# vsergeev/luaradio

Measured on AMD Instinct MI355X. Metric: MSamples/s per block (128-tap complex FIR headline) + WBFM chain end-to-end, higher is better.
Workload: dtype f32

## Files before the change

luaradio_amd/csrc/kernels_channelizer.h:

```cpp
#pragma once
#include "common.h"
#include "kernels_fir.h"

#ifndef LRHIP_CHAN_EXP
#define LRHIP_CHAN_EXP 0
#endif

namespace lrhip {

#ifndef LRHIP_CHAN_INTERLEAVE
#define LRHIP_CHAN_INTERLEAVE 1
#endif
#ifndef LRHIP_CHAN_RT
#define LRHIP_CHAN_RT 1
#endif
#ifndef LRHIP_CHAN_KSLAB
#define LRHIP_CHAN_KSLAB 32
#endif
constexpr int CHAN_RT = LRHIP_CHAN_RT;
constexpr int CHAN_MT = 64 * CHAN_RT;
constexpr int CHAN_KSLAB = LRHIP_CHAN_KSLAB;

template <int NCT>
__global__ __launch_bounds__(256, CHAN_RT == 1 ? 2 : 1) void channelizer_kernel(const float *__restrict__ hist, const float *__restrict__ x,
                                                             const float *__restrict__ W, float *__restrict__ y,
                                                             int M, long n, long nframes, long first)
{
    constexpr int K2 = 16 * NCT;
    constexpr int K = K2 / 2;
    constexpr int DROW = K2 + 2;
    constexpr int WROW = K2 + 16;
    extern __shared__ __attribute__((aligned(16))) float lds[];
    const int tid = threadIdx.x, lane = tid & 63, wave = tid >> 6;
    const int col = lane & 15, kq = lane >> 4;
    const long f0 = (long)blockIdx.x * CHAN_MT;
    const int nsamp = (CHAN_MT - 1) * K + M;
    const int nflt = 2 * nsamp;
    float *ldsD = lds;
    const int dsize = ((nflt + 2 * (nflt / K2) + 2 + 3) / 4) * 4;
    float *ldsW = lds + dsize;

    const long p0 = first + f0 * K;
    const long xlo = p0 - (M - 1);
    if (xlo >= 0 && xlo + nsamp <= n && ((reinterpret_cast<uintptr_t>(x + 2 * xlo) & 15) == 0)) {
        const float4 *src = reinterpret_cast<const float4 *>(x + 2 * xlo);
        for (int i4 = tid; i4 < nflt / 4; i4 += 256) {
            float4 v = src[i4];
            int a = 4 * i4, p = a + 2 * (a / K2);
            *reinterpret_cast<float2 *>(ldsD + p) = make_float2(v.x, v.y);
            *reinterpret_cast<float2 *>(ldsD + p + 2) = make_float2(v.z, v.w);
        }
        for (int a = (nflt / 4) * 4 + tid; a < nflt; a += 256) ldsD[a + 2 * (a / K2)] = x[2 * xlo + a];
    } else {
        for (int r = tid; r < nsamp; r += 256) {
            int a = 2 * r, p = a + 2 * (a / K2);
            ldsD[p] = stream_at<2>(hist, x, p0 + r, 0, M, n);
            ldsD[p + 1] = stream_at<2>(hist, x, p0 + r, 1, M, n);
        }
    }

    constexpr int SLAB_F4 = CHAN_KSLAB * K2 / 4;
    constexpr int UW = (SLAB_F4 + 255) / 256;
    const float4 *W4 = reinterpret_cast<const float4 *>(W);
    static_assert(UW <= 8, "W slab prefetch: at most 8 float4 per thread");
    float4 w0, w1, w2, w3, w4, w5, w6, w7;
#define LR_CHAN_FOR8(OP) OP(0) OP(1) OP(2) OP(3) OP(4) OP(5) OP(6) OP(7)
#define LR_CHAN_LOAD(U)                                                                          \
    if (U < UW) {                                                                                \
        int i4 = tid + U * 256;                                                                  \
        w##U = W4[wbase + (i4 < SLAB_F4 ? i4 : SLAB_F4 - 1)];                                    \
    }
#define LR_CHAN_PUT(U)                                                                           \
    if (U < UW) {                                                                                \
        int i4 = tid + U * 256;                                                                  \
        if (i4 < SLAB_F4) *reinterpret_cast<float4 *>(wdst + ((4 * i4) / K2) * WROW + (4 * i4) % K2) = w##U; \
    }
    {
        const size_t wbase = 0;
        float *wdst = ldsW;
        LR_CHAN_FOR8(LR_CHAN_LOAD)
        LR_CHAN_FOR8(LR_CHAN_PUT)
    }
    __syncthreads();

    f32x4 acc[CHAN_RT][NCT];
#pragma unroll
    for (int r = 0; r < CHAN_RT; r++)
#pragma unroll
        for (int c = 0; c < NCT; c++) acc[r][c] = (f32x4){0.f, 0.f, 0.f, 0.f};
    const float *abase = ldsD + DROW * (wave * 16 * CHAN_RT + col) + kq;
    const int nslabs = 2 * M / CHAN_KSLAB;
    for (int s = 0; s < nslabs; s++) {
        const float *wcur = ldsW + (s & 1) * (CHAN_KSLAB * WROW);
#if LRHIP_CHAN_EXP == 1
        const bool more = false;
#else
        const bool more = s + 1 < nslabs;
#endif
        if (more) {
            const size_t wbase = (size_t)(s + 1) * SLAB_F4;
            LR_CHAN_FOR8(LR_CHAN_LOAD)
        }
        const float *ap = abase + CHAN_KSLAB * s + 2 * ((CHAN_KSLAB * s) / K2);
        const float *bp = wcur + kq * WROW + col;
        constexpr int NST = CHAN_KSLAB / 4;
        float av[2][CHAN_RT], bv[2][NCT];
        auto fetch = [&](int buf, int st) {
#pragma unroll
            for (int r = 0; r < CHAN_RT; r++) av[buf][r] = ap[16 * r * DROW + 4 * st];
#pragma unroll
            for (int c = 0; c < NCT; c++) bv[buf][c] = bp[4 * st * WROW + 16 * c];
        };
        fetch(0, 0);
#pragma unroll
        for (int st = 0; st < NST; st++) {
#if LRHIP_CHAN_INTERLEAVE
            if (st + 1 < NST) fetch((st + 1) & 1, st + 1);
#pragma unroll
            for (int c = 0; c < NCT; c++)
#pragma unroll
                for (int r = 0; r < CHAN_RT; r++)
                    acc[r][c] = __builtin_amdgcn_mfma_f32_16x16x4f32(av[st & 1][r], bv[st & 1][c], acc[r][c], 0, 0, 0);
#pragma unroll
            for (int i = 0; i < NCT * CHAN_RT; i++) {
                __builtin_amdgcn_sched_group_barrier(0x008, 1, 0);
                __builtin_amdgcn_sched_group_barrier(0x100, 1, 0);
            }
            __builtin_amdgcn_sched_barrier(0);
#else
            if (st + 1 < NST) fetch((st + 1) & 1, st + 1);
            __builtin_amdgcn_sched_barrier(0);
#pragma unroll
            for (int c = 0; c < NCT; c++)
#pragma unroll
                for (int r = 0; r < CHAN_RT; r++)
                    acc[r][c] = __builtin_amdgcn_mfma_f32_16x16x4f32(av[st & 1][r], bv[st & 1][c], acc[r][c], 0, 0, 0);
            __builtin_amdgcn_sched_barrier(0);
#endif
        }
        if (more) {
            float *wdst = ldsW + ((s + 1) & 1) * (CHAN_KSLAB * WROW);
            LR_CHAN_FOR8(LR_CHAN_PUT)
        }
#if LRHIP_CHAN_EXP != 1
        __syncthreads();
#endif
    }

#pragma unroll
    for (int rt = 0; rt < CHAN_RT; rt++)
#pragma unroll
        for (int c = 0; c < NCT; c++)
#pragma unroll
            for (int r = 0; r < 4; r++) {
                long f = f0 + (wave * CHAN_RT + rt) * 16 + 4 * kq + r;
                if (f < nframes) y[f * K2 + 16 * c + col] = acc[rt][c][r];
            }
}

#undef LR_CHAN_FOR8
#undef LR_CHAN_LOAD
#undef LR_CHAN_PUT

}
```

luaradio_amd/csrc/lrhip.hip:

```cpp
#include "../../include/lrhip.h"

#include <cmath>
#include <map>
#include <memory>
#include <string>

#include "common.h"
#include "kernels_elem.h"
#include "kernels_fft.h"
#include "kernels_fir.h"
#include "kernels_firfft.h"
#include "kernels_firdecfft.h"
#include "kernels_firdecim.h"
#include "kernels_channelizer.h"
#include "kernels_pfb.h"
#include "kernels_iir.h"
#include "kernels_agc.h"
#include "kernels_firwin.h"
#include "kernels_firwin2.h"
#include "kernels_firfft4k.h"
#include "kernels_firpols.h"
#include "kernels_firfft64.h"
#include "kernels_interp.h"
#include "kernels_rx.h"
#include "kernels_digital.h"
#include "kernels_bitscan.h"
#include "kernels_preamble.h"
#include "kernels_rdsframer.h"
#include "kernels_ertframer.h"
#include "kernels_ax25framer.h"
#include "kernels_pocsagframer.h"
#include "kernels_phasecorr.h"
#include "kernels_modulator.h"
#include "kernels_pll.h"

using namespace lrhip;

static int g_launches = 0;
#define LR_LAUNCH_CHECK()                                                                              \
    do {                                                                                               \
        g_launches++;                                                                                  \
        hipError_t e__ = hipGetLastError();                                                            \
        if (e__ != hipSuccess) return set_error("kernel launch failed: %s (%s:%d)", hipGetErrorString(e__), __FILE__, __LINE__); \
    } while (0)

#include "stage.h"
#include "stage_counted.h"
#include "stage_fir.h"
#include "stage_elem.h"
#include "stage_iir.h"
#include "stage_firwin.h"
#include "stage_spectrum.h"
#include "stage_elem2.h"
#include "stage_resample.h"
#include "stage_pfb.h"
#include "stage_elem3.h"
#include "stage_rx.h"
#include "chain.h"
#include "stage_phasecorr.h"
#include "stage_digital.h"
#include "stage_pll.h"
#include "stage_preamble.h"
#include "stage_framers.h"
#include "stage_modulator.h"
#include "chain_plan.h"

extern "C" {

const char *lrhip_version(void) { return "lrhip 0.1 (gfx950)"; }
const char *lrhip_strerror(void) { return err_buf(); }

int lrhip_init(int device)
{
    err_buf()[0] = 0;
    return ensure_init(device);
}

int lrhip_device(void)
{
    const Context &c = ctx();
    return (c.ready && c.pid == (long)getpid()) ? c.device : -1;
}

int lrhip_device_count(void)
{
    if (ctx().ready && ctx().pid != (long)getpid()) return ensure_init();
    int count = 0;
    LR_HIP(hipGetDeviceCount(&count));
    return count;
}

int lrhip_set_stream(void *hip_stream)
{
    if (ensure_init()) return -1;
    hipStream_t next = hip_stream == (void *)1 ? (hipStream_t) nullptr : hip_stream ? (hipStream_t)hip_stream : ctx().own_stream, prev = ctx().stream;
    if (next != prev) {
        hipEvent_t ev = nullptr;
// ... 284 lines not shown
    if (q->reset()) return nullptr;
    return q.release();
}

lrhip_stage_t *lrhip_unary_create(const char *op, float re, float im, int constant_complex, int input_complex)
{
    if (!op) { set_error("unary: missing operation name"); return nullptr; }
    {
        std::string name;
        std::map<std::string, double> kv;
        const char *c = strchr(op, ':');
        const std::string head(op, c ? (size_t)(c - op) : strlen(op));
        if (head == "preamblesampler") return preamblesampler_create(op);
        if (head == "pam" || head == "qam") return modulator_create(op);
        if (head == "pll") return pll_create(op);
        if (head == "rdsframer") return plain_create<RfStage>(op, 8);
        if (head == "scmframer") return plain_create<EfStage<EF_SCM>>(op, EfProto<EF_SCM>::REC);
        if (head == "scmplusframer") return plain_create<EfStage<EF_SCMPLUS>>(op, EfProto<EF_SCMPLUS>::REC);
        if (head == "idmframer") return plain_create<EfStage<EF_IDM>>(op, EfProto<EF_IDM>::REC);
        if (head == "ax25framer") return plain_create<AxStage>(op, AX_REC);
        if (head == "pocsagframer") return plain_create<PgStage>(op, PG_REC);
        if (head == "manchesterdecoder") {
            if (!parse_op(op, name, kv, {"invert"})) return nullptr;
            return manchesterdecoder_create(kv, op);
        }
        if (c || digital_unary_op(head)) {
            if (!digital_unary_op(head)) { set_error("unary: unknown operation \"%s\"", op); return nullptr; }
            if (!parse_op(op, name, kv, digital_keys(head))) return nullptr;
            return digital_unary_create(name, kv, op);
        }
    }
    struct { const char *name; int code, in, out; } T[] = {
        {"complexmagnitude", UN_CMAG, 8, 4}, {"complexphase", UN_CPHASE, 8, 4}, {"complextoreal", UN_CREAL, 8, 4},
        {"complextoimag", UN_CIMAG, 8, 4},   {"complexconjugate", UN_CCONJ, 8, 8}, {"realtocomplex", UN_R2C, 4, 8},
        {"absolutevalue", UN_ABS, 4, 4}};
    int code = -1, in = 0, out = 0;
    for (auto &t : T)
        if (!strcmp(t.name, op)) { code = t.code; in = t.in; out = t.out; }
    if (!strcmp(op, "addconstant")) {
        if (constant_complex && !input_complex) { set_error("addconstant: a complex constant takes ComplexFloat32 input only (addconstant.lua:42-44)"); return nullptr; }
        code = !input_complex ? UN_ADDC_REAL : (constant_complex ? UN_ADDC_CPLX : UN_ADDC_CPLX_BY_REAL);
        in = out = input_complex ? 8 : 4;
    }
    if (code < 0) { set_error("unary: unknown operation \"%s\"", op); return nullptr; }
    if (ensure_init()) return nullptr;
    UnaryStage *q = new (std::nothrow) UnaryStage();
    if (!q) { set_error("out of memory"); return nullptr; }
    q->op = code; q->cr = re; q->ci = im;
    q->in_size = in; q->out_size = out;
    return q;
}

lrhip_stage_t *lrhip_delay_create(unsigned num_samples, int elem_size)
{
    if (num_samples < 1) { set_error("Number of samples must be greater than 0"); return nullptr; }
    if (elem_size != 4 && elem_size != 8) { set_error("delay: element size must be 4 or 8"); return nullptr; }
    if (ensure_init()) return nullptr;
    std::unique_ptr<DelayStage> q(new (std::nothrow) DelayStage());
    if (!q) { set_error("out of memory"); return nullptr; }
    q->D = num_samples;
    q->in_size = q->out_size = elem_size;
    if (q->reset()) return nullptr;
    return q.release();
}

lrhip_stage_t *lrhip_hilbert_create(const float *taps, unsigned ntaps)
{
    if (!taps || (ntaps % 2) != 1) { set_error("Number of taps must be odd"); return nullptr; }
    std::unique_ptr<HilbertStage> q(new (std::nothrow) HilbertStage());
    if (!q) { set_error("out of memory"); return nullptr; }
    q->fir.reset(fir_build(taps, ntaps, 0, 0, 1, 0, false, 0.0));
    if (!q->fir) return nullptr;
    q->in_size = 4; q->out_size = 8;
    return q.release();
}

lrhip_stage_t *lrhip_channelizer_create(const float *taps, unsigned ntaps, unsigned nchannels)
{
    if (!taps || ntaps < 32 || (ntaps % 32) != 0 || ntaps > 8192) { set_error("channelizer: ntaps must be a multiple of 32 in [32, 8192]"); return nullptr; }
    if (nchannels != 32 && nchannels != 64) { set_error("channelizer: nchannels must be 32 or 64"); return nullptr; }
    if (ensure_init()) return nullptr;
    std::unique_ptr<ChannelizerStage> q(new (std::nothrow) ChannelizerStage());
    if (!q) { set_error("out of memory"); return nullptr; }
    int M = (int)ntaps, K = (int)nchannels, K2 = 2 * K;
    q->M = M; q->K = K;
    q->in_size = q->out_size = 8;
    std::vector<float> W((size_t)2 * M * K2);
    const double PI2 = 6.283185307179586476925286766559;
    for (int i = 0; i < M; i++)
        for (int c = 0; c < K; c++) {
            int j = M - 1 - i;
            double a = PI2 * (double)(((long)c * j) % K) / K, h = taps[j];
            float gr = (float)(h * std::cos(a)), gi = (float)(h * std::sin(a));
            W[(size_t)(2 * i) * K2 + 2 * c] = gr;
            W[(size_t)(2 * i + 1) * K2 + 2 * c] = -gi;
            W[(size_t)(2 * i) * K2 + 2 * c + 1] = gi;
            W[(size_t)(2 * i + 1) * K2 + 2 * c + 1] = gr;
        }
    if (upload(q->W, W.data(), W.size() * sizeof(float))) return nullptr;
    if (q->reset()) return nullptr;
    return q.release();
}

lrhip_stage_t *lrhip_pfb_channelizer_create(const float *taps, unsigned ntaps, unsigned nchannels)
{
    return lrhip_pfb_oversampled_create(taps, ntaps, nchannels, 1);
}

lrhip_stage_t *lrhip_pfb_oversampled_create(const float *taps, unsigned ntaps, unsigned nchannels, unsigned oversample)
{
    if (const char *why = PfbChannelizerStage::refusal(taps ? ntaps : 0, nchannels, oversample)) { set_error("%s", why); return nullptr; }
    if (ensure_init()) return nullptr;
    std::unique_ptr<PfbChannelizerStage> q(new (std::nothrow) PfbChannelizerStage());
    if (!q) { set_error("out of memory"); return nullptr; }
    const int M = (int)ntaps, K = (int)nchannels;
    q->M = M; q->K = K; q->P = (M + K - 1) / K;
    q->R = (int)oversample; q->D = K / q->R;
    while ((1 << q->log2k) < K) q->log2k++;
    q->in_size = q->out_size = 8;
    std::vector<float> tw((size_t)K);
    for (int m = 0; m < K / 2; m++) {
        double ang = -2.0 * 3.14159265358979323846 * m / K;
        tw[2 * m] = (float)std::cos(ang);
        tw[2 * m + 1] = (float)std::sin(ang);
    }
    if (upload(q->taps, taps, (size_t)M * sizeof(float)) || upload(q->tw, tw.data(), tw.size() * sizeof(float))) return nullptr;
    if (q->reset()) return nullptr;
    return q.release();
}

lrhip_stage_t *lrhip_binary_create(const char *op, int input_complex)
{
    if (!op) { set_error("binary: missing operation name"); return nullptr; }
    if (!strcmp(op, "sampler")) {
        if (ensure_init()) return nullptr;
        std::unique_ptr<SamplerStage> q(new (std::nothrow) SamplerStage());
        if (!q) { set_error("out of memory"); return nullptr; }
        q->in_size = q->out_size = input_complex ? 8 : 4;
        q->in2_size = 4;
        if (q->reset()) return nullptr;
        return q.release();
    }
    int code = !strcmp(op, "multiply") ? BIN_MULTIPLY : !strcmp(op, "multiplyconjugate") ? BIN_MULTIPLY_CONJ
             : !strcmp(op, "add") ? BIN_ADD : !strcmp(op, "subtract") ? BIN_SUBTRACT : !strcmp(op, "floattocomplex") ? BIN_F2C : -1;
    if (code < 0) { set_error("binary: unknown operation \"%s\"", op); return nullptr; }
    if (code == BIN_MULTIPLY_CONJ && !input_complex) { set_error("binary: multiplyconjugate takes ComplexFloat32 inputs (multiplyconjugate.lua:26)"); return nullptr; }
    if (ensure_init()) return nullptr;
    BinaryStage *q = new (std::nothrow) BinaryStage();
    if (!q) { set_error("out of memory"); return nullptr; }
    q->op = code;
    q->in_size = q->out_size = input_complex ? 8 : 4;
    if (code == BIN_F2C) { q->in_size = 4; q->out_size = 8; }
    return q;
}

void lrhip_stage_destroy(lrhip_stage_t *q)
{
    if (!q) return;
    if (ctx().ready) (void)hipStreamSynchronize(ctx().stream);
    delete q;
}

int lrhip_stage_reset(lrhip_stage_t *q) { return q ? q->reset() : set_error("null stage"); }
int lrhip_stage_input_size(const lrhip_stage_t *q) { return q ? q->in_size : set_error("null stage"); }
int lrhip_stage_output_size(const lrhip_stage_t *q) { return q ? q->out_size : set_error("null stage"); }
unsigned long lrhip_stage_max_output(const lrhip_stage_t *q, unsigned long n_in) { return q ? q->max_output(n_in) : 0; }

long lrhip_stage_execute_device(lrhip_stage_t *q, const void *in_dev, unsigned long n_in, void *out_dev, unsigned long out_capacity)
{
    if (!q) return set_error("null stage");
    if (n_in && (!in_dev || (!out_dev && q->max_output(n_in)))) return set_error("null buffer");
    return q->run(in_dev, n_in, out_dev, out_capacity);
}

long lrhip_stage_execute(lrhip_stage_t *q, const void *in_host, unsigned long n_in, void *out_host, unsigned long out_capacity)
{
    if (!q) return set_error("null stage");
    return host_execute(q->h_in, q->h_out, q->d_in, q->d_out, q->in_size, q->out_size, q->max_output(n_in), in_host, n_in,
                        out_host, out_capacity,
                        [&](const void *di, unsigned long n, void *dout, unsigned long cap) { return q->run(di, n, dout, cap); }, q->align(), q->direct_io_ok());
}
// ... 770 lines not shown
```

luaradio_amd/csrc/stage_resample.h:

```cpp
#pragma once

struct ResampleStage : lrhip_stage {
    int S = 2, M = 0, L = 1, HQ = 0;
    unsigned long D = 1;
    float c = 1.f;
    DeviceBuf d_taps, d_ttab, hist[2];
    int cur = 0;
    uint64_t Q0 = 0, m0 = 0;
    int interp_J = 0;
    int rat_blocks_per_cu = 0;
    static bool rational_supported(int L, unsigned long D) { return (L == 3 && D == 2) || (L == 2 && D == 3) || (L == 4 && D == 3) || (L == 3 && D == 4) || (L == 5 && D == 4) || (L == 4 && D == 5); }
    int interp_blocks_per_cu = 0;
    static int resample_rounds(long ntiles, long slots)
    {
        static const char *e = getenv("LRHIP_RESAMPLE_ROUNDS");
        if (e) return atoi(e) < 0 ? 0 : atoi(e);
        return ntiles <= slots ? 0 : 1;
    }
    static constexpr int SPAN_MAX = 6144;
    const char *kind() const override { return "resample"; }
    unsigned long max_output(unsigned long n) const override { return (n * (unsigned long)L) / D + 2; }
    int seek(unsigned long long n0, unsigned long long *n0_out) override
    {
        if (reset()) return -1;
// ... 26 lines not shown
                if (!interp_blocks_per_cu) {
                    int nb = 0;
                    LR_HIP(hipOccupancyMaxActiveBlocksPerMultiprocessor(&nb, kern, FIP_NT, lds_bytes));
                    interp_blocks_per_cu = nb < 1 ? 1 : nb;
                }
                const long ntiles = ((long)n + tq - 1) / tq, slots = (long)ctx().num_cus * interp_blocks_per_cu;
                const int rounds = resample_rounds(ntiles, slots);
                const long wgs = rounds > 0 ? (ntiles + rounds - 1) / rounds : (ntiles < slots ? ntiles : slots);
                hipLaunchKernelGGL(kern, dim3((unsigned)wgs), dim3(FIP_NT), lds_bytes, ctx().stream, h, (const float *)in_dev, (const float *)d_ttab.p,
                                   (float *)out_dev, (long)n, HQ, c, ho, ablation_bits("LRHIP_INTERP_DBG"), rounds);
                return 0;
            };
#define LR_INTERP(LL, JJ) gi(fir_interp_kernel<LL, JJ>, (size_t)FipGeom<LL, JJ>::LDS_FLOATS * sizeof(float), FipGeom<LL, JJ>::TQ)
            int rc = L == 2 ? LR_INTERP(2, 64) : L == 3 ? LR_INTERP(3, 43) : L == 4 ? LR_INTERP(4, 32) : LR_INTERP(5, 26);
#undef LR_INTERP
            if (rc) return rc;
            LR_LAUNCH_CHECK();
            cur ^= 1;
            Q0 += n;
            m0 = m_end;
            return n_out;
        }
        static const bool no_rational = getenv("LRHIP_NO_RATIONAL_WIN") != nullptr;
        if (!no_rational && interp_J > 0 && D > 1 && ((uintptr_t)in_dev & 7) == 0 && ((uintptr_t)out_dev & 7) == 0) {
            auto gr = [&](auto kern, size_t lds_bytes, int tq) -> int {
                if (lds_bytes > 48 * 1024) LR_HIP(hipFuncSetAttribute((const void *)kern, hipFuncAttributeMaxDynamicSharedMemorySize, (int)lds_bytes));
                if (!rat_blocks_per_cu) {
                    int nb = 0;
                    LR_HIP(hipOccupancyMaxActiveBlocksPerMultiprocessor(&nb, kern, 256, lds_bytes));
                    rat_blocks_per_cu = nb < 1 ? 1 : nb;
                }
                const long ntiles = ((long)n + (long)(Q0 % D) + tq - 1) / tq, slots = (long)ctx().num_cus * rat_blocks_per_cu;
                const int rounds = resample_rounds(ntiles, slots);
                const long wgs = rounds > 0 ? (ntiles + rounds - 1) / rounds : (ntiles < slots ? ntiles : slots);
                hipLaunchKernelGGL(kern, dim3((unsigned)wgs), dim3(256), lds_bytes, ctx().stream, h, (const float *)in_dev, (const float *)d_ttab.p,
                                   (float *)out_dev, (long)n, n_out, m0, Q0, HQ, c, ho, rounds);
                return 0;
            };
#define LR_RAT(LL, DD, JJ, RR) gr(fir_rational_kernel<LL, DD, JJ, RR>, (size_t)FrrGeom<LL, DD, JJ, RR>::LDS_FLOATS * sizeof(float), FrrGeom<LL, DD, JJ, RR>::TQ)
            int rc = (L == 3 && D == 2) ? LR_RAT(3, 2, 43, 6) : (L == 2 && D == 3) ? LR_RAT(2, 3, 64, 9) : (L == 4 && D == 3) ? LR_RAT(4, 3, 32, 6)
                   : (L == 3 && D == 4) ? LR_RAT(3, 4, 43, 8) : (L == 5 && D == 4) ? LR_RAT(5, 4, 26, 8) : LR_RAT(4, 5, 32, 10);
#undef LR_RAT
            if (rc) return rc;
            LR_LAUNCH_CHECK();
            cur ^= 1;
            Q0 += n;
            m0 = m_end;
            return n_out;
        }
        int span_cap = (int)(256 * D / (unsigned long)L) + (M - 1) / L + 4;
        size_t lds_bytes = ((size_t)((((M - 1) / L + 1) * L + 3) & ~3) + (size_t)span_cap * S) * sizeof(float);
        auto go = [&](auto kern) -> int {
            if (lds_bytes > 48 * 1024) LR_HIP(hipFuncSetAttribute((const void *)kern, hipFuncAttributeMaxDynamicSharedMemorySize, (int)lds_bytes));
            unsigned grid = n_out > 0 ? (unsigned)((n_out + 255) / 256) : 1;
            hipLaunchKernelGGL(kern, dim3(grid), dim3(256), lds_bytes, ctx().stream, h, (const float *)in_dev, (const float *)d_taps.p, (float *)out_dev, M, L,
                               (long)D, (long)n, n_out, m0, Q0, HQ, c, span_cap, ho);
            return 0;
        };
        int rc = S == 2 ? go(fir_resample_kernel<2>) : go(fir_resample_kernel<1>);
        if (rc) return rc;
        LR_LAUNCH_CHECK();
        cur ^= 1;
        Q0 += n;
        m0 = m_end;
        return n_out;
    }
};

struct ChannelizerStage : lrhip_stage {
    int seek(unsigned long long, unsigned long long *) override { return set_error("seek: not supported by the channelizer stage"); }
    long memory() const override { return -1; }
    int M = 0, K = 0;
    DeviceBuf W, hist[2];
    int cur = 0;
    unsigned long index = 0;
    const char *kind() const override { return "channelizer"; }
    unsigned long max_output(unsigned long n) const override { return (n / K + 1) * K; }
    int reset() override
    {
        cur = 0; index = 0;
        size_t hb = (size_t)(M - 1) * 2 * sizeof(float);
        return (zero_fill(hist[0], hb) || zero_fill(hist[1], hb)) ? -1 : 0;
    }
    template <int NCT>
    int launch(const float *x, long n, float *y, long nframes)
    {
        constexpr int K2 = 16 * NCT;
        int nflt = 2 * ((CHAN_MT - 1) * K + M);
        size_t dsize = (size_t)((nflt + 2 * (nflt / K2) + 2 + 3) / 4) * 4;
        size_t lds_bytes = (dsize + (size_t)2 * CHAN_KSLAB * (K2 + 16)) * sizeof(float);
        auto kern = channelizer_kernel<NCT>;
        if (lds_bytes > 48 * 1024) LR_HIP(hipFuncSetAttribute((const void *)kern, hipFuncAttributeMaxDynamicSharedMemorySize, (int)lds_bytes));
        unsigned grid = (unsigned)((nframes + CHAN_MT - 1) / CHAN_MT);
        hipLaunchKernelGGL(kern, dim3(grid), dim3(256), lds_bytes, ctx().stream, (const float *)hist[cur].p, x, (const float *)W.p, y, M, n,
                           nframes, (long)index);
        LR_LAUNCH_CHECK();
        return 0;
    }
    long run(const void *in_dev, unsigned long n_in, void *out_dev, unsigned long cap) override
    {
        long n = (long)n_in;
        if (n <= 0) return 0;
        long nframes = n_in > index ? (long)((n_in - index + K - 1) / K) : 0;
        if ((unsigned long)(nframes * K) > cap) return set_error("channelizer: output capacity %lu < %ld", cap, nframes * K);
        const float *x = (const float *)in_dev;
        if (nframes > 0) {
            int rc = K == 32 ? launch<4>(x, n, (float *)out_dev, nframes) : launch<8>(x, n, (float *)out_dev, nframes);
            if (rc) return rc;
        }
        unsigned grid = grid_for((unsigned long)(M - 1) * 2, 256);
        hipLaunchKernelGGL(fir_history_kernel<2>, dim3(grid), dim3(256), 0, ctx().stream, (const float *)hist[cur].p, x, (float *)hist[cur ^ 1].p, M, n);
        LR_LAUNCH_CHECK();
        cur ^= 1;
        index = index + (unsigned long)nframes * K - n_in;
        return nframes * K;
    }
};
```

Before: 317,200.

## Split channelizer input into Re/Im planes and exploit real-DFT symmetry for half-size GEMM

The channelizer now splits interleaved complex input into separate real and imaginary LDS planes. It multiplies each plane by a real K-column weight matrix that holds cos for channels 0..K/2 and sin for channels 1..K/2-1, instead of a 2K-wide complex-expanded matrix. The epilogue rebuilds channels c and K-c from the four partial sums, which halves the weight matrix and the MFMA work per frame. In exchange it requires ntaps to be a multiple of the slab size and removes the multi-row-tile option.

Result: no change. 317,400, median of 3 (+0.1%).

```diff
diff --git a/luaradio_amd/csrc/kernels_channelizer.h b/luaradio_amd/csrc/kernels_channelizer.h
--- a/luaradio_amd/csrc/kernels_channelizer.h
+++ b/luaradio_amd/csrc/kernels_channelizer.h
@@ -11,60 +11,67 @@
 #ifndef LRHIP_CHAN_INTERLEAVE
 #define LRHIP_CHAN_INTERLEAVE 1
 #endif
-#ifndef LRHIP_CHAN_RT
-#define LRHIP_CHAN_RT 1
-#endif
 #ifndef LRHIP_CHAN_KSLAB
 #define LRHIP_CHAN_KSLAB 32
 #endif
-constexpr int CHAN_RT = LRHIP_CHAN_RT;
-constexpr int CHAN_MT = 64 * CHAN_RT;
+constexpr int CHAN_MT = 64;
 constexpr int CHAN_KSLAB = LRHIP_CHAN_KSLAB;
 
+__host__ __device__ constexpr int chan_tile_samples(int K, int M) { return (CHAN_MT - 1) * K + M; }
+__host__ __device__ constexpr int chan_plane_floats(int K, int M)
+{
+    return (chan_tile_samples(K, M) + 2 * (chan_tile_samples(K, M) / K) + 2 + 3) / 4 * 4;
+}
+__host__ __device__ constexpr int chan_wrow(int K) { return K + 16; }
+__host__ __device__ constexpr size_t chan_lds_bytes(int K, int M)
+{
+    return ((size_t)2 * chan_plane_floats(K, M) + (size_t)2 * CHAN_KSLAB * chan_wrow(K)) * sizeof(float);
+}
+
 template <int NCT>
-__global__ __launch_bounds__(256, CHAN_RT == 1 ? 2 : 1) void channelizer_kernel(const float *__restrict__ hist, const float *__restrict__ x,
+__global__ __launch_bounds__(256, 2) void channelizer_kernel(const float *__restrict__ hist, const float *__restrict__ x,
                                                              const float *__restrict__ W, float *__restrict__ y,
                                                              int M, long n, long nframes, long first)
 {
-    constexpr int K2 = 16 * NCT;
-    constexpr int K = K2 / 2;
-    constexpr int DROW = K2 + 2;
-    constexpr int WROW = K2 + 16;
+    constexpr int K = 16 * NCT;
+    constexpr int H = NCT / 2;
+    constexpr int DROW = K + 2;
+    constexpr int WROW = chan_wrow(K);
+    static_assert(NCT % 2 == 0, "Re and Im of a channel sit in tiles t and t + NCT/2");
+    static_assert(K % CHAN_KSLAB == 0 || CHAN_KSLAB % K == 0, "a slab starts on a plane row or stays inside one");
     extern __shared__ __attribute__((aligned(16))) float lds[];
     const int tid = threadIdx.x, lane = tid & 63, wave = tid >> 6;
     const int col = lane & 15, kq = lane >> 4;
     const long f0 = (long)blockIdx.x * CHAN_MT;
-    const int nsamp = (CHAN_MT - 1) * K + M;
-    const int nflt = 2 * nsamp;
-    float *ldsD = lds;
-    const int dsize = ((nflt + 2 * (nflt / K2) + 2 + 3) / 4) * 4;
-    float *ldsW = lds + dsize;
+    const int nsamp = chan_tile_samples(K, M);
+    const int psize = chan_plane_floats(K, M);
+    float *ldsRe = lds, *ldsIm = lds + psize;
+    float *ldsW = lds + 2 * psize;
 
     const long p0 = first + f0 * K;
     const long xlo = p0 - (M - 1);
     if (xlo >= 0 && xlo + nsamp <= n && ((reinterpret_cast<uintptr_t>(x + 2 * xlo) & 15) == 0)) {
         const float4 *src = reinterpret_cast<const float4 *>(x + 2 * xlo);
-        for (int i4 = tid; i4 < nflt / 4; i4 += 256) {
+        for (int i4 = tid; i4 < nsamp / 2; i4 += 256) {
             float4 v = src[i4];
-            int a = 4 * i4, p = a + 2 * (a / K2);
-            *reinterpret_cast<float2 *>(ldsD + p) = make_float2(v.x, v.y);
-            *reinterpret_cast<float2 *>(ldsD + p + 2) = make_float2(v.z, v.w);
+            int r = 2 * i4, p = r + 2 * (r / K);
+            *reinterpret_cast<float2 *>(ldsRe + p) = make_float2(v.x, v.z);
+            *reinterpret_cast<float2 *>(ldsIm + p) = make_float2(v.y, v.w);
         }
-        for (int a = (nflt / 4) * 4 + tid; a < nflt; a += 256) ldsD[a + 2 * (a / K2)] = x[2 * xlo + a];
     } else {
         for (int r = tid; r < nsamp; r += 256) {
-            int a = 2 * r, p = a + 2 * (a / K2);
-            ldsD[p] = stream_at<2>(hist, x, p0 + r, 0, M, n);
-            ldsD[p + 1] = stream_at<2>(hist, x, p0 + r, 1, M, n);
+            int p = r + 2 * (r / K);
+            ldsRe[p] = stream_at<2>(hist, x, p0 + r, 0, M, n);
+            ldsIm[p] = stream_at<2>(hist, x, p0 + r, 1, M, n);
         }
     }
 
-    constexpr int SLAB_F4 = CHAN_KSLAB * K2 / 4;
+    constexpr int SLAB_F4 = CHAN_KSLAB * K / 4;
     constexpr int UW = (SLAB_F4 + 255) / 256;
     const float4 *W4 = reinterpret_cast<const float4 *>(W);
-    static_assert(UW <= 8, "W slab prefetch: at most 8 float4 per thread");
-    float4 w0, w1, w2, w3, w4, w5, w6, w7;
-#define LR_CHAN_FOR8(OP) OP(0) OP(1) OP(2) OP(3) OP(4) OP(5) OP(6) OP(7)
+    static_assert(UW <= 4, "G slab prefetch: at most 4 float4 per thread");
+    float4 w0, w1, w2, w3;
+#define LR_CHAN_FOR4(OP) OP(0) OP(1) OP(2) OP(3)
 #define LR_CHAN_LOAD(U)                                                                          \
     if (U < UW) {                                                                                \
         int i4 = tid + U * 256;                                                                  \
@@ -73,23 +80,23 @@
 #define LR_CHAN_PUT(U)                                                                           \
     if (U < UW) {                                                                                \
         int i4 = tid + U * 256;                                                                  \
-        if (i4 < SLAB_F4) *reinterpret_cast<float4 *>(wdst + ((4 * i4) / K2) * WROW + (4 * i4) % K2) = w##U; \
+        if (i4 < SLAB_F4) *reinterpret_cast<float4 *>(wdst + ((4 * i4) / K) * WROW + (4 * i4) % K) = w##U; \
     }
     {
         const size_t wbase = 0;
         float *wdst = ldsW;
-        LR_CHAN_FOR8(LR_CHAN_LOAD)
-        LR_CHAN_FOR8(LR_CHAN_PUT)
+        LR_CHAN_FOR4(LR_CHAN_LOAD)
+        LR_CHAN_FOR4(LR_CHAN_PUT)
     }
     __syncthreads();
 
-    f32x4 acc[CHAN_RT][NCT];
+    f32x4 acc[2][NCT];
 #pragma unroll
-    for (int r = 0; r < CHAN_RT; r++)
+    for (int p = 0; p < 2; p++)
 #pragma unroll
-        for (int c = 0; c < NCT; c++) acc[r][c] = (f32x4){0.f, 0.f, 0.f, 0.f};
-    const float *abase = ldsD + DROW * (wave * 16 * CHAN_RT + col) + kq;
-    const int nslabs = 2 * M / CHAN_KSLAB;
+        for (int c = 0; c < NCT; c++) acc[p][c] = (f32x4){0.f, 0.f, 0.f, 0.f};
+    const float *abase = ldsRe + DROW * (wave * 16 + col) + kq;
+    const int nslabs = M / CHAN_KSLAB;
     for (int s = 0; s < nslabs; s++) {
         const float *wcur = ldsW + (s & 1) * (CHAN_KSLAB * WROW);
 #if LRHIP_CHAN_EXP == 1
@@ -99,15 +106,15 @@
 #endif
         if (more) {
             const size_t wbase = (size_t)(s + 1) * SLAB_F4;
-            LR_CHAN_FOR8(LR_CHAN_LOAD)
+            LR_CHAN_FOR4(LR_CHAN_LOAD)
         }
-        const float *ap = abase + CHAN_KSLAB * s + 2 * ((CHAN_KSLAB * s) / K2);
+        const float *ap = abase + CHAN_KSLAB * s + 2 * ((CHAN_KSLAB * s) / K);
         const float *bp = wcur + kq * WROW + col;
         constexpr int NST = CHAN_KSLAB / 4;
-        float av[2][CHAN_RT], bv[2][NCT];
+        float av[2][2], bv[2][NCT];
         auto fetch = [&](int buf, int st) {
-#pragma unroll
-            for (int r = 0; r < CHAN_RT; r++) av[buf][r] = ap[16 * r * DROW + 4 * st];
+            av[buf][0] = ap[4 * st + 2 * ((4 * st) / K)];
+            av[buf][1] = ap[4 * st + 2 * ((4 * st) / K) + psize];
 #pragma unroll
             for (int c = 0; c < NCT; c++) bv[buf][c] = bp[4 * st * WROW + 16 * c];
         };
@@ -119,10 +126,10 @@
 #pragma unroll
             for (int c = 0; c < NCT; c++)
 #pragma unroll
-                for (int r = 0; r < CHAN_RT; r++)
-                    acc[r][c] = __builtin_amdgcn_mfma_f32_16x16x4f32(av[st & 1][r], bv[st & 1][c], acc[r][c], 0, 0, 0);
+                for (int p = 0; p < 2; p++)
+                    acc[p][c] = __builtin_amdgcn_mfma_f32_16x16x4f32(av[st & 1][p], bv[st & 1][c], acc[p][c], 0, 0, 0);
 #pragma unroll
-            for (int i = 0; i < NCT * CHAN_RT; i++) {
+            for (int i = 0; i < 2 * NCT; i++) {
                 __builtin_amdgcn_sched_group_barrier(0x008, 1, 0);
                 __builtin_amdgcn_sched_group_barrier(0x100, 1, 0);
             }
@@ -133,32 +140,40 @@
 #pragma unroll
             for (int c = 0; c < NCT; c++)
 #pragma unroll
-                for (int r = 0; r < CHAN_RT; r++)
-                    acc[r][c] = __builtin_amdgcn_mfma_f32_16x16x4f32(av[st & 1][r], bv[st & 1][c], acc[r][c], 0, 0, 0);
+                for (int p = 0; p < 2; p++)
+                    acc[p][c] = __builtin_amdgcn_mfma_f32_16x16x4f32(av[st & 1][p], bv[st & 1][c], acc[p][c], 0, 0, 0);
             __builtin_amdgcn_sched_barrier(0);
 #endif
         }
         if (more) {
             float *wdst = ldsW + ((s + 1) & 1) * (CHAN_KSLAB * WROW);
-            LR_CHAN_FOR8(LR_CHAN_PUT)
+            LR_CHAN_FOR4(LR_CHAN_PUT)
         }
 #if LRHIP_CHAN_EXP != 1
         __syncthreads();
 #endif
     }
 
+    float2 *y2 = reinterpret_cast<float2 *>(y);
 #pragma unroll
-    for (int rt = 0; rt < CHAN_RT; rt++)
+    for (int t = 0; t < H; t++)
 #pragma unroll
-        for (int c = 0; c < NCT; c++)
-#pragma unroll
-            for (int r = 0; r < 4; r++) {
-                long f = f0 + (wave * CHAN_RT + rt) * 16 + 4 * kq + r;
-                if (f < nframes) y[f * K2 + 16 * c + col] = acc[rt][c][r];
+        for (int r = 0; r < 4; r++) {
+            const long f = f0 + wave * 16 + 4 * kq + r;
+            if (f >= nframes) continue;
+            const int c = 16 * t + col;
+            const float Rr = acc[0][t][r], Ir = acc[1][t][r], Ri = acc[0][t + H][r], Ii = acc[1][t + H][r];
+            if (c != 0) {
+                y2[f * K + c] = make_float2(Rr - Ii, Ir + Ri);
+                y2[f * K + (K - c)] = make_float2(Rr + Ii, Ir - Ri);
+            } else {
+                y2[f * K] = make_float2(Rr + 0.f * Ir, Ir + 0.f * Rr);
+                y2[f * K + K / 2] = make_float2(Ri + 0.f * Ii, Ii + 0.f * Ri);
             }
+        }
 }
 
-#undef LR_CHAN_FOR8
+#undef LR_CHAN_FOR4
 #undef LR_CHAN_LOAD
 #undef LR_CHAN_PUT
 
diff --git a/luaradio_amd/csrc/lrhip.hip b/luaradio_amd/csrc/lrhip.hip
--- a/luaradio_amd/csrc/lrhip.hip
+++ b/luaradio_amd/csrc/lrhip.hip
@@ -463,20 +463,17 @@
     if (ensure_init()) return nullptr;
     std::unique_ptr<ChannelizerStage> q(new (std::nothrow) ChannelizerStage());
     if (!q) { set_error("out of memory"); return nullptr; }
-    int M = (int)ntaps, K = (int)nchannels, K2 = 2 * K;
+    int M = (int)ntaps, K = (int)nchannels, Kh = K / 2;
     q->M = M; q->K = K;
     q->in_size = q->out_size = 8;
-    std::vector<float> W((size_t)2 * M * K2);
+    std::vector<float> W((size_t)M * K);
     const double PI2 = 6.283185307179586476925286766559;
     for (int i = 0; i < M; i++)
-        for (int c = 0; c < K; c++) {
+        for (int c = 0; c <= Kh; c++) {
             int j = M - 1 - i;
             double a = PI2 * (double)(((long)c * j) % K) / K, h = taps[j];
-            float gr = (float)(h * std::cos(a)), gi = (float)(h * std::sin(a));
-            W[(size_t)(2 * i) * K2 + 2 * c] = gr;
-            W[(size_t)(2 * i + 1) * K2 + 2 * c] = -gi;
-            W[(size_t)(2 * i) * K2 + 2 * c + 1] = gi;
-            W[(size_t)(2 * i + 1) * K2 + 2 * c + 1] = gr;
+            W[(size_t)i * K + c] = (float)(h * std::cos(a));
+            if (c >= 1 && c < Kh) W[(size_t)i * K + Kh + c] = (float)(h * std::sin(a));
         }
     if (upload(q->W, W.data(), W.size() * sizeof(float))) return nullptr;
     if (q->reset()) return nullptr;
diff --git a/luaradio_amd/csrc/stage_resample.h b/luaradio_amd/csrc/stage_resample.h
--- a/luaradio_amd/csrc/stage_resample.h
+++ b/luaradio_amd/csrc/stage_resample.h
@@ -135,10 +135,8 @@
     template <int NCT>
     int launch(const float *x, long n, float *y, long nframes)
     {
-        constexpr int K2 = 16 * NCT;
-        int nflt = 2 * ((CHAN_MT - 1) * K + M);
-        size_t dsize = (size_t)((nflt + 2 * (nflt / K2) + 2 + 3) / 4) * 4;
-        size_t lds_bytes = (dsize + (size_t)2 * CHAN_KSLAB * (K2 + 16)) * sizeof(float);
+        if (M % CHAN_KSLAB) return set_error("channelizer: ntaps %d is not a multiple of the %d-row slab this library was built with", M, CHAN_KSLAB);
+        size_t lds_bytes = chan_lds_bytes(16 * NCT, M);
         auto kern = channelizer_kernel<NCT>;
         if (lds_bytes > 48 * 1024) LR_HIP(hipFuncSetAttribute((const void *)kern, hipFuncAttributeMaxDynamicSharedMemorySize, (int)lds_bytes));
         unsigned grid = (unsigned)((nframes + CHAN_MT - 1) / CHAN_MT);
@@ -155,7 +153,7 @@
         if ((unsigned long)(nframes * K) > cap) return set_error("channelizer: output capacity %lu < %ld", cap, nframes * K);
         const float *x = (const float *)in_dev;
         if (nframes > 0) {
-            int rc = K == 32 ? launch<4>(x, n, (float *)out_dev, nframes) : launch<8>(x, n, (float *)out_dev, nframes);
+            int rc = K == 32 ? launch<2>(x, n, (float *)out_dev, nframes) : launch<4>(x, n, (float *)out_dev, nframes);
             if (rc) return rc;
         }
         unsigned grid = grid_for((unsigned long)(M - 1) * 2, 256);
```

## Use conjugate-symmetric paired DFT table with split real/imag planes in channelizer

Applied to the files above, without the earlier changes.

Replaces the channelizer's complex GEMM, which used a 2x-expanded interleaved real/imag weight matrix, with a paired cos/sin table of K columns. Input is deinterleaved into separate real and imaginary LDS planes. Outputs for channel c and K-c are reconstructed from four real partial sums. This roughly halves the MFMA count and the weight traffic per frame. The cost is a larger LDS footprint for the two planes and a more complex epilogue that writes output in scattered pairs.

Measured after the change: 315,900 before, 315,800 after (median of 2 runs). No clear change (-0.0%).

```diff
diff --git a/luaradio_amd/csrc/channelizer_table.h b/luaradio_amd/csrc/channelizer_table.h
--- /dev/null
+++ b/luaradio_amd/csrc/channelizer_table.h
@@ -0,0 +1,25 @@
+#pragma once
+#include <cmath>
+#include <cstddef>
+#include <vector>
+
+namespace lrhip {
+
+inline std::vector<float> channelizer_paired_table(const float *taps, int M, int K)
+{
+    std::vector<float> Wp((size_t)M * K);
+    const double PI2 = 6.283185307179586476925286766559;
+    const int H = K / 2;
+    for (int i = 0; i < M; i++) {
+        const int j = M - 1 - i;
+        const double h = taps[j];
+        float *row = Wp.data() + (size_t)i * K;
+        auto angle = [&](int c) { return PI2 * (double)(((long)c * j) % K) / K; };
+        for (int c = 0; c < H; c++) row[c] = (float)(h * std::cos(angle(c)));
+        row[H] = (float)(h * std::cos(angle(H)));
+        for (int c = 1; c < H; c++) row[H + c] = (float)(h * std::sin(angle(c)));
+    }
+    return Wp;
+}
+
+}
diff --git a/luaradio_amd/csrc/kernels_channelizer.h b/luaradio_amd/csrc/kernels_channelizer.h
--- a/luaradio_amd/csrc/kernels_channelizer.h
+++ b/luaradio_amd/csrc/kernels_channelizer.h
@@ -2,69 +2,62 @@
 #include "common.h"
 #include "kernels_fir.h"
 
-#ifndef LRHIP_CHAN_EXP
-#define LRHIP_CHAN_EXP 0
-#endif
-
 namespace lrhip {
 
-#ifndef LRHIP_CHAN_INTERLEAVE
-#define LRHIP_CHAN_INTERLEAVE 1
-#endif
-#ifndef LRHIP_CHAN_RT
-#define LRHIP_CHAN_RT 1
-#endif
-#ifndef LRHIP_CHAN_KSLAB
-#define LRHIP_CHAN_KSLAB 32
-#endif
-constexpr int CHAN_RT = LRHIP_CHAN_RT;
-constexpr int CHAN_MT = 64 * CHAN_RT;
-constexpr int CHAN_KSLAB = LRHIP_CHAN_KSLAB;
+constexpr int CHAN_MT = 64;
+constexpr int CHAN_KSLAB = 32;
 
-template <int NCT>
-__global__ __launch_bounds__(256, CHAN_RT == 1 ? 2 : 1) void channelizer_kernel(const float *__restrict__ hist, const float *__restrict__ x,
-                                                             const float *__restrict__ W, float *__restrict__ y,
+__host__ __device__ constexpr int chan_plane_floats(int nsamp, int K) { return ((nsamp + 2 * (nsamp / K) + 2 + 3) / 4) * 4; }
+__host__ __device__ constexpr size_t chan_lds_floats(int M, int K)
+{
+    return (size_t)2 * chan_plane_floats((CHAN_MT - 1) * K + M, K) + (size_t)2 * CHAN_KSLAB * (K + 16);
+}
+
+template <int NT>
+__global__ __launch_bounds__(256, 2) void channelizer_kernel(const float *__restrict__ hist, const float *__restrict__ x,
+                                                             const float *__restrict__ Wp, float *__restrict__ y,
                                                              int M, long n, long nframes, long first)
 {
-    constexpr int K2 = 16 * NCT;
-    constexpr int K = K2 / 2;
-    constexpr int DROW = K2 + 2;
-    constexpr int WROW = K2 + 16;
+    constexpr int K = 16 * NT;
+    constexpr int HT = NT / 2;
+    constexpr int DROW = K + 2;
+    constexpr int WROW = K + 16;
+    static_assert(NT == 2 || NT == 4, "K is 32 or 64");
+    static_assert(CHAN_KSLAB % 4 == 0 && K % CHAN_KSLAB == 0, "a slab lies inside one plane row");
     extern __shared__ __attribute__((aligned(16))) float lds[];
     const int tid = threadIdx.x, lane = tid & 63, wave = tid >> 6;
     const int col = lane & 15, kq = lane >> 4;
     const long f0 = (long)blockIdx.x * CHAN_MT;
     const int nsamp = (CHAN_MT - 1) * K + M;
-    const int nflt = 2 * nsamp;
-    float *ldsD = lds;
-    const int dsize = ((nflt + 2 * (nflt / K2) + 2 + 3) / 4) * 4;
-    float *ldsW = lds + dsize;
+    const int psize = chan_plane_floats(nsamp, K);
+    float *ldsA = lds;
+    float *ldsB = lds + psize;
+    float *ldsW = lds + 2 * psize;
 
     const long p0 = first + f0 * K;
     const long xlo = p0 - (M - 1);
     if (xlo >= 0 && xlo + nsamp <= n && ((reinterpret_cast<uintptr_t>(x + 2 * xlo) & 15) == 0)) {
         const float4 *src = reinterpret_cast<const float4 *>(x + 2 * xlo);
-        for (int i4 = tid; i4 < nflt / 4; i4 += 256) {
-            float4 v = src[i4];
-            int a = 4 * i4, p = a + 2 * (a / K2);
-            *reinterpret_cast<float2 *>(ldsD + p) = make_float2(v.x, v.y);
-            *reinterpret_cast<float2 *>(ldsD + p + 2) = make_float2(v.z, v.w);
+        for (int i2 = tid; i2 < nsamp / 2; i2 += 256) {
+            float4 v = src[i2];
+            int r = 2 * i2, p = r + 2 * (r / K);
+            *reinterpret_cast<float2 *>(ldsA + p) = make_float2(v.x, v.z);
+            *reinterpret_cast<float2 *>(ldsB + p) = make_float2(v.y, v.w);
         }
-        for (int a = (nflt / 4) * 4 + tid; a < nflt; a += 256) ldsD[a + 2 * (a / K2)] = x[2 * xlo + a];
     } else {
         for (int r = tid; r < nsamp; r += 256) {
-            int a = 2 * r, p = a + 2 * (a / K2);
-            ldsD[p] = stream_at<2>(hist, x, p0 + r, 0, M, n);
-            ldsD[p + 1] = stream_at<2>(hist, x, p0 + r, 1, M, n);
+            int p = r + 2 * (r / K);
+            ldsA[p] = stream_at<2>(hist, x, p0 + r, 0, M, n);
+            ldsB[p] = stream_at<2>(hist, x, p0 + r, 1, M, n);
         }
     }
 
-    constexpr int SLAB_F4 = CHAN_KSLAB * K2 / 4;
+    constexpr int SLAB_F4 = CHAN_KSLAB * K / 4;
     constexpr int UW = (SLAB_F4 + 255) / 256;
-    const float4 *W4 = reinterpret_cast<const float4 *>(W);
-    static_assert(UW <= 8, "W slab prefetch: at most 8 float4 per thread");
-    float4 w0, w1, w2, w3, w4, w5, w6, w7;
-#define LR_CHAN_FOR8(OP) OP(0) OP(1) OP(2) OP(3) OP(4) OP(5) OP(6) OP(7)
+    const float4 *W4 = reinterpret_cast<const float4 *>(Wp);
+    static_assert(UW <= 2, "Wp slab prefetch: at most 2 float4 per thread");
+    float4 w0, w1;
+#define LR_CHAN_FOR2(OP) OP(0) OP(1)
 #define LR_CHAN_LOAD(U)                                                                          \
     if (U < UW) {                                                                                \
         int i4 = tid + U * 256;                                                                  \
@@ -73,92 +66,86 @@
 #define LR_CHAN_PUT(U)                                                                           \
     if (U < UW) {                                                                                \
         int i4 = tid + U * 256;                                                                  \
-        if (i4 < SLAB_F4) *reinterpret_cast<float4 *>(wdst + ((4 * i4) / K2) * WROW + (4 * i4) % K2) = w##U; \
+        if (i4 < SLAB_F4) *reinterpret_cast<float4 *>(wdst + ((4 * i4) / K) * WROW + (4 * i4) % K) = w##U; \
     }
     {
         const size_t wbase = 0;
         float *wdst = ldsW;
-        LR_CHAN_FOR8(LR_CHAN_LOAD)
-        LR_CHAN_FOR8(LR_CHAN_PUT)
+        LR_CHAN_FOR2(LR_CHAN_LOAD)
+        LR_CHAN_FOR2(LR_CHAN_PUT)
     }
     __syncthreads();
 
-    f32x4 acc[CHAN_RT][NCT];
+    f32x4 acc[2][NT];
 #pragma unroll
-    for (int r = 0; r < CHAN_RT; r++)
+    for (int pl = 0; pl < 2; pl++)
 #pragma unroll
-        for (int c = 0; c < NCT; c++) acc[r][c] = (f32x4){0.f, 0.f, 0.f, 0.f};
-    const float *abase = ldsD + DROW * (wave * 16 * CHAN_RT + col) + kq;
-    const int nslabs = 2 * M / CHAN_KSLAB;
+        for (int t = 0; t < NT; t++) acc[pl][t] = (f32x4){0.f, 0.f, 0.f, 0.f};
+    const int aoff = DROW * (wave * 16 + col) + kq;
+    const int nslabs = M / CHAN_KSLAB;
     for (int s = 0; s < nslabs; s++) {
         const float *wcur = ldsW + (s & 1) * (CHAN_KSLAB * WROW);
-#if LRHIP_CHAN_EXP == 1
-        const bool more = false;
-#else
         const bool more = s + 1 < nslabs;
-#endif
         if (more) {
             const size_t wbase = (size_t)(s + 1) * SLAB_F4;
-            LR_CHAN_FOR8(LR_CHAN_LOAD)
+            LR_CHAN_FOR2(LR_CHAN_LOAD)
         }
-        const float *ap = abase + CHAN_KSLAB * s + 2 * ((CHAN_KSLAB * s) / K2);
+        const int i0 = CHAN_KSLAB * s;
+        const float *apA = ldsA + aoff + i0 + 2 * (i0 / K);
+        const float *apB = ldsB + aoff + i0 + 2 * (i0 / K);
         const float *bp = wcur + kq * WROW + col;
         constexpr int NST = CHAN_KSLAB / 4;
-        float av[2][CHAN_RT], bv[2][NCT];
+        float av[2][2], bv[2][NT];
         auto fetch = [&](int buf, int st) {
+            av[buf][0] = apA[4 * st];
+            av[buf][1] = apB[4 * st];
 #pragma unroll
-            for (int r = 0; r < CHAN_RT; r++) av[buf][r] = ap[16 * r * DROW + 4 * st];
-#pragma unroll
-            for (int c = 0; c < NCT; c++) bv[buf][c] = bp[4 * st * WROW + 16 * c];
+            for (int t = 0; t < NT; t++) bv[buf][t] = bp[4 * st * WROW + 16 * t];
         };
         fetch(0, 0);
 #pragma unroll
         for (int st = 0; st < NST; st++) {
-#if LRHIP_CHAN_INTERLEAVE
             if (st + 1 < NST) fetch((st + 1) & 1, st + 1);
 #pragma unroll
-            for (int c = 0; c < NCT; c++)
+            for (int t = 0; t < NT; t++)
 #pragma unroll
-                for (int r = 0; r < CHAN_RT; r++)
-                    acc[r][c] = __builtin_amdgcn_mfma_f32_16x16x4f32(av[st & 1][r], bv[st & 1][c], acc[r][c], 0, 0, 0);
+                for (int pl = 0; pl < 2; pl++)
+                    acc[pl][t] = __builtin_amdgcn_mfma_f32_16x16x4f32(av[st & 1][pl], bv[st & 1][t], acc[pl][t], 0, 0, 0);
 #pragma unroll
-            for (int i = 0; i < NCT * CHAN_RT; i++) {
+            for (int i = 0; i < 2 * NT; i++) {
                 __builtin_amdgcn_sched_group_barrier(0x008, 1, 0);
                 __builtin_amdgcn_sched_group_barrier(0x100, 1, 0);
             }
             __builtin_amdgcn_sched_barrier(0);
-#else
-            if (st + 1 < NST) fetch((st + 1) & 1, st + 1);
-            __builtin_amdgcn_sched_barrier(0);
-#pragma unroll
-            for (int c = 0; c < NCT; c++)
-#pragma unroll
-                for (int r = 0; r < CHAN_RT; r++)
-                    acc[r][c] = __builtin_amdgcn_mfma_f32_16x16x4f32(av[st & 1][r], bv[st & 1][c], acc[r][c], 0, 0, 0);
-            __builtin_amdgcn_sched_barrier(0);
-#endif
         }
         if (more) {
             float *wdst = ldsW + ((s + 1) & 1) * (CHAN_KSLAB * WROW);
-            LR_CHAN_FOR8(LR_CHAN_PUT)
+            LR_CHAN_FOR2(LR_CHAN_PUT)
         }
-#if LRHIP_CHAN_EXP != 1
         __syncthreads();
-#endif
     }
 
+    float2 *y2 = reinterpret_cast<float2 *>(y);
 #pragma unroll
-    for (int rt = 0; rt < CHAN_RT; rt++)
+    for (int t = 0; t < HT; t++) {
+        const int c = 16 * t + col;
 #pragma unroll
-        for (int c = 0; c < NCT; c++)
-#pragma unroll
-            for (int r = 0; r < 4; r++) {
-                long f = f0 + (wave * CHAN_RT + rt) * 16 + 4 * kq + r;
-                if (f < nframes) y[f * K2 + 16 * c + col] = acc[rt][c][r];
+        for (int r = 0; r < 4; r++) {
+            const long f = f0 + wave * 16 + 4 * kq + r;
+            if (f >= nframes) continue;
+            const float S1 = acc[0][t][r], S4 = acc[1][t][r], S3 = acc[0][HT + t][r], S2 = acc[1][HT + t][r];
+            if (c == 0) {
+                y2[f * K] = make_float2(S1 + 0.0f * S4, S4 + 0.0f * S1);
+                y2[f * K + K / 2] = make_float2(S3 + 0.0f * S2, S2 + 0.0f * S3);
+            } else {
+                y2[f * K + c] = make_float2(S1 - S2, S3 + S4);
+                y2[f * K + K - c] = make_float2(S1 + S2, S4 - S3);
             }
+        }
+    }
 }
 
-#undef LR_CHAN_FOR8
+#undef LR_CHAN_FOR2
 #undef LR_CHAN_LOAD
 #undef LR_CHAN_PUT
 
diff --git a/luaradio_amd/csrc/lrhip.hip b/luaradio_amd/csrc/lrhip.hip
--- a/luaradio_amd/csrc/lrhip.hip
+++ b/luaradio_amd/csrc/lrhip.hip
@@ -13,6 +13,7 @@
 #include "kernels_firdecfft.h"
 #include "kernels_firdecim.h"
 #include "kernels_channelizer.h"
+#include "channelizer_table.h"
 #include "kernels_pfb.h"
 #include "kernels_iir.h"
 #include "kernels_agc.h"
@@ -463,21 +464,10 @@
     if (ensure_init()) return nullptr;
     std::unique_ptr<ChannelizerStage> q(new (std::nothrow) ChannelizerStage());
     if (!q) { set_error("out of memory"); return nullptr; }
-    int M = (int)ntaps, K = (int)nchannels, K2 = 2 * K;
+    int M = (int)ntaps, K = (int)nchannels;
     q->M = M; q->K = K;
     q->in_size = q->out_size = 8;
-    std::vector<float> W((size_t)2 * M * K2);
-    const double PI2 = 6.283185307179586476925286766559;
-    for (int i = 0; i < M; i++)
-        for (int c = 0; c < K; c++) {
-            int j = M - 1 - i;
-            double a = PI2 * (double)(((long)c * j) % K) / K, h = taps[j];
-            float gr = (float)(h * std::cos(a)), gi = (float)(h * std::sin(a));
-            W[(size_t)(2 * i) * K2 + 2 * c] = gr;
-            W[(size_t)(2 * i + 1) * K2 + 2 * c] = -gi;
-            W[(size_t)(2 * i) * K2 + 2 * c + 1] = gi;
-            W[(size_t)(2 * i + 1) * K2 + 2 * c + 1] = gr;
-        }
+    const std::vector<float> W = channelizer_paired_table(taps, M, K);
     if (upload(q->W, W.data(), W.size() * sizeof(float))) return nullptr;
     if (q->reset()) return nullptr;
     return q.release();
diff --git a/luaradio_amd/csrc/stage_resample.h b/luaradio_amd/csrc/stage_resample.h
--- a/luaradio_amd/csrc/stage_resample.h
+++ b/luaradio_amd/csrc/stage_resample.h
@@ -132,14 +132,11 @@
         size_t hb = (size_t)(M - 1) * 2 * sizeof(float);
         return (zero_fill(hist[0], hb) || zero_fill(hist[1], hb)) ? -1 : 0;
     }
-    template <int NCT>
+    template <int NT>
     int launch(const float *x, long n, float *y, long nframes)
     {
-        constexpr int K2 = 16 * NCT;
-        int nflt = 2 * ((CHAN_MT - 1) * K + M);
-        size_t dsize = (size_t)((nflt + 2 * (nflt / K2) + 2 + 3) / 4) * 4;
-        size_t lds_bytes = (dsize + (size_t)2 * CHAN_KSLAB * (K2 + 16)) * sizeof(float);
-        auto kern = channelizer_kernel<NCT>;
+        size_t lds_bytes = chan_lds_floats(M, 16 * NT) * sizeof(float);
+        auto kern = channelizer_kernel<NT>;
         if (lds_bytes > 48 * 1024) LR_HIP(hipFuncSetAttribute((const void *)kern, hipFuncAttributeMaxDynamicSharedMemorySize, (int)lds_bytes));
         unsigned grid = (unsigned)((nframes + CHAN_MT - 1) / CHAN_MT);
         hipLaunchKernelGGL(kern, dim3(grid), dim3(256), lds_bytes, ctx().stream, (const float *)hist[cur].p, x, (const float *)W.p, y, M, n,
@@ -155,7 +152,7 @@
         if ((unsigned long)(nframes * K) > cap) return set_error("channelizer: output capacity %lu < %ld", cap, nframes * K);
         const float *x = (const float *)in_dev;
         if (nframes > 0) {
-            int rc = K == 32 ? launch<4>(x, n, (float *)out_dev, nframes) : launch<8>(x, n, (float *)out_dev, nframes);
+            int rc = K == 32 ? launch<2>(x, n, (float *)out_dev, nframes) : launch<4>(x, n, (float *)out_dev, nframes);
             if (rc) return rc;
         }
         unsigned grid = grid_for((unsigned long)(M - 1) * 2, 256);
```
